# driskai/scenario_gym

Measured on NVIDIA B200. Metric: entity-steps/s, batched rollout+collision, higher is better.
Workload: dtype f64

## Files before the change

### scenario_gym_b200/csrc/sg_common.cuh

```cuda
#pragma once
#include <cuda_runtime.h>
#include <math.h>
#include <stdio.h>
#include <string.h>

#include "sg_device.cuh"
#include "sg_layout.h"

static __constant__ double c_ngon[64][2] = {
#include "sg_ngon.inc"
};

struct Grp {
  int n, s, M, G, W, H, QCAP, bar_id;
  unsigned mask;
  int64_t i, nm;
  double* corners;
  double* actbuf;
  double* rbox;
  unsigned corners_sh, rbox_sh;
  double* tcold;
  double* hcs;
  double* pedbuf;
  float4* pednb;
  uint16_t* nblist;
  double* boxp;
  double* egop;
  double* cold_d;
  int* cold_i;
  float4* aabb;
  uint32_t* queue;
  uint32_t* ego_now;
  uint32_t* ego_last;
  uint32_t* bits;
  int* acc;
  uint8_t* flags;
  int8_t* orient;
  uint16_t* sid;
  uint16_t* posof;
  int* sflag;
  float* skey;
  float4* tmpbox;
  int sorted;
  uint32_t* gstart;
  uint16_t* gsorted;
  uint16_t* glarge;
  int* gmisc;
};

SG_DEV void cp_async8(unsigned smem_addr, const void* gsrc) {
  asm volatile("cp.async.ca.shared.global [%0], [%1], 8;" ::"r"(smem_addr), "l"(gsrc) : "memory");
}
SG_DEV void cp_async_commit() { asm volatile("cp.async.commit_group;" ::: "memory"); }
SG_DEV void cp_async_wait_all() { asm volatile("cp.async.wait_group 0;" ::: "memory"); }

SG_DEV void group_sync(const Grp& g) {
  if (g.G <= 32) __syncwarp(g.mask);
  else asm volatile("bar.sync %0, %1;" ::"r"(g.bar_id), "r"(g.G) : "memory");
}

SG_DEV void setup_group(Grp& g, const SgScene& sc, const GroupLayout& L, unsigned char* smem,
                        int gl, int s, int n, int M = -1) {
  if (M < 0) M = sc.n_slots;
  unsigned char* base = smem + (size_t)gl * L.bytes;
  g.n = n; g.s = s; g.M = M; g.G = L.G; g.W = L.W; g.H = L.H; g.QCAP = L.QCAP;
  g.bar_id = 1 + gl;
  g.mask = 0xffffffffu;
  if (L.G < 32) g.mask = ((1u << L.G) - 1u) << ((threadIdx.x & 31) / L.G * L.G);
  g.nm = sc.plane_stride;
  g.i = (int64_t)n * M + s;
  g.corners = (double*)base;
  g.actbuf = (double*)(base + L.off_act);
  g.rbox = (double*)(base + L.off_rbox);
  g.corners_sh = (unsigned)__cvta_generic_to_shared(base);
  g.rbox_sh = g.corners_sh + (unsigned)L.off_rbox;
  g.tcold = (double*)(base + L.off_tcold);
  g.hcs = (double*)(base + L.off_hcs);
  g.pedbuf = (double*)(base + L.off_ped);
  g.pednb = (float4*)(base + L.off_pednb);
  g.nblist = (uint16_t*)(base + L.off_nbl);
  g.boxp = (double*)(base + L.off_box);
  g.egop = (double*)(base + L.off_ego);
  g.cold_d = (double*)(base + L.off_cold);
  g.cold_i = (int*)(base + L.off_cold + COLD_ND * sizeof(double));
  g.aabb = (float4*)(base + L.off_aabb);
  g.queue = (uint32_t*)(base + L.off_queue);
  g.ego_now = (uint32_t*)(base + L.off_hits);
  g.ego_last = g.ego_now + L.W;
  g.bits = (uint32_t*)(base + L.off_bits);
  g.acc = (int*)(base + L.off_acc);
  g.flags = (uint8_t*)(base + L.off_flags);
  g.orient = (int8_t*)(base + L.off_orient);
  g.sid = (uint16_t*)(base + L.off_sid);
  g.posof = (uint16_t*)(base + L.off_posof);
  g.sflag = (int*)(base + L.off_sflag);
  g.skey = (float*)(base + L.off_skey) + SG_SORT_WIN + 1;
  g.tmpbox = (float4*)(base + L.off_tmpbox);
  g.sorted = L.sorted;
  g.gstart = (uint32_t*)(base + L.off_gstart);
  g.gsorted = (uint16_t*)(base + L.off_gsorted);
  g.glarge = (uint16_t*)(base + L.off_glarge);
  g.gmisc = (int*)(base + L.off_gmisc);
}

SG_DEV double fast_rcp(double d) {
  double r;
  asm("rcp.approx.ftz.f64 %0, %1;" : "=d"(r) : "d"(d));
  double e = __fma_rn(-d, r, 1.0);
  r = __fma_rn(r, e, r);
  e = __fma_rn(-d, r, 1.0);
  return __fma_rn(r, e, r);
}

SG_DEV double fast_sqrt(double x) {
  double y;
  asm("rsqrt.approx.ftz.f64 %0, %1;" : "=d"(y) : "d"(x));
  const double hx = 0.5 * x;
  double e = __fma_rn(-hx * y, y, 0.5);
  y = __fma_rn(y, e, y);
  e = __fma_rn(-hx * y, y, 0.5);
  y = __fma_rn(y, e, y);
  double r = x * y;
  r = __fma_rn(__fma_rn(-r, r, x), 0.5 * y, r);
  return x > 0.0 ? r : 0.0;
}
SG_DEV double fnorm2(double a, double b) { return fast_sqrt(a * a + b * b); }

SG_DEV double div_r(double n, double d, double r) {
  const double q = n * r;
  const double rem = __fma_rn(-q, d, n);
  return __fma_rn(rem, r, q);
}

SG_DEV float4 make_aabb_box(double x, double y, double cs, double sn, double bw, double bl,
                            double bcx, double bcy, double ox, double oy) {
  const double xc = x + (bcx * cs - bcy * sn), yc = y + (bcx * sn + bcy * cs);
  const double hl = 0.5 * bl, hw = 0.5 * bw;
  const double m = 3.552713678800501e-15 *
                   (fabs(x) + fabs(y) + fabs(bl) + fabs(bw) + fabs(bcx) + fabs(bcy));
  const double ex = fabs(hl * cs) + fabs(hw * sn) + m, ey = fabs(hl * sn) + fabs(hw * cs) + m;
  float4 b;
  b.x = __double2float_rd(__dsub_rd(__dsub_rd(xc, ex), ox));
  b.y = __double2float_rd(__dsub_rd(__dsub_rd(yc, ey), oy));
  b.z = __double2float_ru(__dsub_ru(__dadd_ru(xc, ex), ox));
  b.w = __double2float_ru(__dsub_ru(__dadd_ru(yc, ey), oy));
  return b;
}

SG_DEV double min2(double a, double b) { return a < b ? a : b; }
SG_DEV double max2(double a, double b) { return a > b ? a : b; }
SG_DEV double clipd(double v, double lo, double hi) { return v < lo ? lo : (v > hi ? hi : v); }

static __constant__ double c_trig[12] = {
    -1.66666666666666324348e-01, 8.33333333332248946124e-03,  -1.98412698298579493134e-04,
    2.75573137070700676789e-06,  -2.50507602534068634195e-08, 1.58969099521155010221e-10,
    4.16666666666666019037e-02,  -1.38888888888741095749e-03, 2.48015872894767294178e-05,
    -2.75573143513906633035e-07, 2.08757232129817482790e-09,  -1.13596475577881948265e-11};
SG_DEV void sincos_kernel(double x, double& sn, double& cs) {
  const double z = x * x;
  const double* S = c_trig;
  const double* C = c_trig + 6;
  double r = __fma_rn(z, S[5], S[4]);
  r = __fma_rn(z, r, S[3]);
  r = __fma_rn(z, r, S[2]);
  r = __fma_rn(z, r, S[1]);
  r = __fma_rn(z, r, S[0]);
  sn = __fma_rn(x * z, r, x);
  double q = __fma_rn(z, C[5], C[4]);
  q = __fma_rn(z, q, C[3]);
  q = __fma_rn(z, q, C[2]);
  q = __fma_rn(z, q, C[1]);
  q = __fma_rn(z, q, C[0]);
  const double hz = 0.5 * z, w = 1.0 - hz;
  cs = w + (((1.0 - w) - hz) + z * (z * q));
}
static __device__ __noinline__ double2 sincos_lib(double x) {
  double2 r;
  sincos(x, &r.x, &r.y);
  return r;
}
static __device__ __noinline__ double tan_lib(double x) { return tan(x); }

SG_DEV double tan_small(double x) {
  double sn, cs;
  sincos_kernel(x, sn, cs);
  return div_r(sn, cs, fast_rcp(cs));
}
SG_DEV void sincos_fast(double x, double& sn, double& cs) {
  if (!(fabs(x) < 1.0e9)) { const double2 r = sincos_lib(x); sn = r.x; cs = r.y; return; }
  const double kd = rint(x * 0.63661977236758138);
  double r = __fma_rn(-kd, 1.5707963267948966, x);
  r = __fma_rn(-kd, 6.123233995736766e-17, r);
  r = __fma_rn(-kd, -1.4973849048591698e-33, r);
  double a, b;
  sincos_kernel(r, a, b);
  const int k = (int)kd;
  const double s0 = (k & 1) ? b : a, c0 = (k & 1) ? a : b;
  sn = (k & 2) ? -s0 : s0;
  cs = ((k + 1) & 2) ? -c0 : c0;
}

static __device__ __noinline__ bool in_buffer_band(double x, double y, double r, double qx, double qy) {
  const double a = atan2(-(qy - y), qx - x);
  double kk = a * (64.0 / (2.0 * M_PI));
  if (kk < 0.0) kk += 64.0;
  const int k0 = (int)kk;
#pragma unroll 1
  for (int j = -1; j <= 1; ++j) {
    const int k = (k0 + j) & 63, k1 = (k + 1) & 63;
    const double ax = x + r * c_ngon[k][0], ay = y + r * c_ngon[k][1];
    const double bx = x + r * c_ngon[k1][0], by = y + r * c_ngon[k1][1];
    if (orient_sign(ax, ay, bx, by, qx, qy) >= 0) return false;
  }
  return true;
}
SG_DEV bool in_buffer(double x, double y, double r, double qx, double qy) {
  const double dx = qx - x, dy = qy - y, d2 = dx * dx + dy * dy;
  const double rin = r * 0.99879545620517241 * (1.0 - 1e-9);
  if (d2 < rin * rin) return true;
  const double rout = r * (1.0 + 1e-9);
  if (d2 > rout * rout) return false;
  return in_buffer_band(x, y, r, qx, qy);
}

#define SG_AABB_TEST(hits, mb, ob, bit)                                                         \
  asm("{ .reg .pred p;\n\t"                                                                     \
      "setp.le.f32 p, %1, %2;\n\t"                                                              \
      "setp.le.and.f32 p, %3, %4, p;\n\t"                                                       \
      "setp.le.and.f32 p, %5, %6, p;\n\t"                                                       \
      "setp.le.and.f32 p, %7, %8, p;\n\t"                                                       \
      "@p or.b32 %0, %0, %9; }"                                                                  \
      : "+r"(hits)                                                                              \
      : "f"(mb.x), "f"(ob.z), "f"(ob.x), "f"(mb.z), "f"(mb.y), "f"(ob.w), "f"(ob.y), "f"(mb.w), \
        "r"(bit))

SG_DEV void stage_ped_state(const Grp& c, bool present, int etype, double x, double y, double vx,
                            double vy, double r, double ox, double oy) {
  c.flags[c.s] = (uint8_t)((present ? 1 : 0) | (etype << 1));
  c.pedbuf[c.s] = x; c.pedbuf[c.G + c.s] = y;
  c.pedbuf[2 * c.G + c.s] = vx; c.pedbuf[3 * c.G + c.s] = vy;
  float4 b = make_float4(INFINITY, INFINITY, -INFINITY, -INFINITY);
  if (present && etype == SG_ETYPE_PEDESTRIAN) {
    const double h = 0.5 * r * (1.0 + 1e-9);
    b.x = __double2float_rd(__dsub_rd(__dsub_rd(x, h), ox));
    b.y = __double2float_rd(__dsub_rd(__dsub_rd(y, h), oy));
    b.z = __double2float_ru(__dsub_ru(__dadd_ru(x, h), ox));
    b.w = __double2float_ru(__dsub_ru(__dadd_ru(y, h), oy));
  }
  c.pednb[c.s] = b;
}


struct GridPos {
  int ix, iy;
  bool large;
};

SG_DEV uint32_t grid_start(const uint32_t* gs, int cell) {
  const uint32_t w = gs[cell >> 1];
  return (cell & 1) ? (w >> 16) : (w & 0xffffu);
}

SG_DEV int grid_row_ranges(const uint32_t* gs, int ix, int iy, int dy, int beg[2], int end[2]) {
  const int row = ((iy + dy) & (SG_GRID_DIM - 1)) << SG_GRID_BITS;
  const int a = (ix - 1) & (SG_GRID_DIM - 1), b = (ix + 1) & (SG_GRID_DIM - 1);
  if (a < b) {
    beg[0] = (int)grid_start(gs, row | a); end[0] = (int)grid_start(gs, (row | b) + 1);
    return 1;
  }
  beg[0] = (int)grid_start(gs, row | a); end[0] = (int)grid_start(gs, row + SG_GRID_DIM);
  beg[1] = (int)grid_start(gs, row);     end[1] = (int)grid_start(gs, (row | b) + 1);
  return 2;
}

SG_DEV GridPos grid_build(const Grp& c, bool present, bool have_box, double x, double y, double ox,
                          double oy, double cs, double inv_cs) {
  uint32_t* gs = c.gstart;
  const int nwords = SG_GRID_CELLS / 2;
  for (int q = c.s; q <= nwords; q += c.G) gs[q] = 0;
  if (c.s == 0) c.gmisc[0] = 0;
  group_sync(c);
  GridPos g;
  g.ix = 0; g.iy = 0; g.large = false;
  int cell = 0;
  uint32_t rank = 0;
  if (present) {
    const double px = x - ox, py = y - oy;
    g.ix = __double2int_rd(px * inv_cs);
    g.iy = __double2int_rd(py * inv_cs);
    cell = ((g.iy & (SG_GRID_DIM - 1)) << SG_GRID_BITS) | (g.ix & (SG_GRID_DIM - 1));
    if (have_box) {
      const float4 bb = c.aabb[c.s];
      const double reach = fmax(fmax(px - (double)bb.x, (double)bb.z - px),
                                fmax(py - (double)bb.y, (double)bb.w - py));
      g.large = !(reach <= 0.5 * cs * (1.0 - 1e-6));
      if (g.large) {
        const int k = atomicAdd(&c.gmisc[0], 1);
        if (k < SG_GRID_LCAP) c.glarge[k] = (uint16_t)c.s;
      }
    }
    const uint32_t old = atomicAdd(&gs[cell >> 1], (cell & 1) ? 0x10000u : 1u);
    rank = (cell & 1) ? (old >> 16) : (old & 0xffffu);
  }
  group_sync(c);
  const int wpt = (nwords + c.G - 1) / c.G;
  const int w0 = c.s * wpt;
  uint32_t local = 0;
  for (int q = 0; q < wpt; ++q)
    if (w0 + q < nwords) { const uint32_t v = gs[w0 + q]; local += (v & 0xffffu) + (v >> 16); }
  const int lane = threadIdx.x & 31, wid = c.s >> 5;
  uint32_t incl = local;
#pragma unroll
  for (int d = 1; d < 32; d <<= 1) {
    const uint32_t o = __shfl_up_sync(0xffffffffu, incl, d);
    if (lane >= d) incl += o;
  }
  if (lane == 31) c.gmisc[8 + wid] = (int)incl;
  group_sync(c);
  uint32_t wt = lane < (c.G >> 5) ? (uint32_t)c.gmisc[8 + lane] : 0u, wi = wt;
#pragma unroll
  for (int d = 1; d < 32; d <<= 1) {
    const uint32_t o = __shfl_up_sync(0xffffffffu, wi, d);
    if (lane >= d) wi += o;
  }
  const uint32_t wbase = __shfl_sync(0xffffffffu, wi - wt, wid);
  const uint32_t total = __shfl_sync(0xffffffffu, wi, 31);
  uint32_t run = wbase + incl - local;
  for (int q = 0; q < wpt; ++q)
    if (w0 + q < nwords) {
      const uint32_t v = gs[w0 + q], lo = v & 0xffffu, hi = v >> 16;
      gs[w0 + q] = run | ((run + lo) << 16);
      run += lo + hi;
    }
  if (c.s == 0) gs[nwords] = total;
  group_sync(c);
  if (present)
    c.gsorted[grid_start(gs, cell) + rank] = (uint16_t)((uint32_t)c.s | (g.large ? SG_GRID_LARGE : 0u));
  group_sync(c);
  return g;
}

SG_DEV void broad_phase(const Grp& c, int parity);
SG_DEV void broad_phase_grid(const Grp& c, int parity, const GridPos& g) {
  const int nl = c.gmisc[0];
  if (nl > SG_GRID_LCAP) { broad_phase(c, parity); return; }
  const float4 mb = c.aabb[c.s];
  int* acc = c.acc + parity * ACC_N;
  auto test = [&](int o) {
    const float4 ob = c.aabb[o];
    if (mb.x <= ob.z && ob.x <= mb.z && mb.y <= ob.w && ob.y <= mb.w) {
      const int q = atomicAdd(&acc[ACC_QCOUNT], 1);
      if (q < c.QCAP) c.queue[q] = ((uint32_t)c.s << 16) | (uint32_t)o;
    }
  };
  if (!g.large) {
    for (int dy = -1; dy <= 1; ++dy) {
      int beg[2], end[2];
      const int nr = grid_row_ranges(c.gstart, g.ix, g.iy, dy, beg, end);
      for (int r = 0; r < nr; ++r)
        for (int idx = beg[r]; idx < end[r]; ++idx) {
          const uint32_t o = c.gsorted[idx];
          if (o > (uint32_t)c.s && o < SG_GRID_LARGE) test((int)o);
        }
    }
  }
  for (int k = 0; k < nl; ++k) {
    const int o = c.glarge[k];
    if (o == c.s || (g.large && o < c.s)) continue;
    test(o);
  }
}

struct NbForce {
  int valid;
  double a0, a1, b0, b1;
};
SG_DEV NbForce neighbour_force(const SgParams& p, const Grp& c, double px, double py, int o, double step_dt,
                               double sh, double ch, double sight_cos) {
  NbForce f;
  f.valid = 0; f.a0 = 0.0; f.a1 = 0.0; f.b0 = 0.0; f.b1 = 0.0;
  const double* bx = c.pedbuf;
  const double* by = c.pedbuf + c.G;
  const double* bvx = c.pedbuf + 2 * c.G;
  const double* bvy = c.pedbuf + 3 * c.G;
  const double ox = bx[o], oy = by[o];
  if (!in_buffer(px, py, p.ped_distance_threshold, ox, oy)) return f;
  f.valid = 1;
  const double ovx = bvx[o], ovy = bvy[o];
  const double vdx = ovx * ch + ovy * -sh, vdy = ovx * sh + ovy * ch;
  const double vn = fnorm2(vdx, vdy) + 0.0000000001, rvn = fast_rcp(vn);
  const double view0 = div_r(vdx, vn, rvn), view1 = div_r(vdy, vn, rvn);
  const double rx = px - ox, ry = py - oy, rn = fnorm2(rx, ry), rrn = fast_rcp(rn);
  const double vmag = fnorm2(ovx, ovy) + 0.0000000001, rvm = fast_rcp(vmag);
  const double uox = div_r(ovx, vmag, rvm), uoy = div_r(ovy, vmag, rvm);
  const double other_step = vmag * step_dt;
  const double r2x = rx - other_step * uox, r2y = ry - other_step * uoy;
  const double r2n = fnorm2(r2x, r2y) + 0.0000000001, rr2 = fast_rcp(r2n);
  const double b = (1.0 / 2) * fast_sqrt((rn + r2n) * (rn + r2n) - other_step * other_step);
  const double c0 = (1.0 / 4) * fast_rcp(b) * (rn + r2n);
  const double dbx = c0 * (div_r(rx, rn, rrn) + div_r(r2x, r2n, rr2)),
// ... 951 lines not shown
```

### scenario_gym_b200/csrc/sg_layout.h

```cpp
#pragma once
#include <stdint.h>
#include <cuda_runtime.h>

#define SG_THREADS 256
#define SG_NBCAP 12
#ifndef SG_SORT_MIN_M
#define SG_SORT_MIN_M 129
#endif
#ifndef SG_SWEEP_WIN
#define SG_SWEEP_WIN 4
#endif
#ifndef SG_SORT_WIN
#define SG_SORT_WIN 4
#endif
#ifndef SG_WARP_PAIRS
#define SG_WARP_PAIRS 6
#endif
#define SG_GRID_BITS 6
#define SG_GRID_DIM (1 << SG_GRID_BITS)
#define SG_GRID_CELLS (SG_GRID_DIM * SG_GRID_DIM)
#define SG_GRID_LCAP 64
#define SG_GRID_LARGE 0x8000u
#ifndef SG_VEH_THREADS
#define SG_VEH_THREADS 128
#endif
#ifndef SG_VEH_MINB
#define SG_VEH_MINB 4
#endif

struct GroupLayout {
  int G;
  int W;
  int H;
  int QCAP;
  int off_act, off_rbox, off_tcold, off_hcs, off_ped, off_pednb, off_nbl, off_box, off_ego, off_cold, off_aabb, off_queue, off_hits, off_bits,
      off_acc, off_flags, off_orient;
  int sorted;
  int off_sid, off_posof, off_sflag, off_skey, off_tmpbox;
  int grid;
  int off_gstart, off_gsorted, off_glarge, off_gmisc;
  int bytes;
};

enum { EGO_X = 0, EGO_Y, EGO_C, EGO_S, EGO_INV0, EGO_INV1, EGO_HD0, EGO_HD1, EGO_HINV0, EGO_HINV1,
       EGO_V0, EGO_V1, EGO_VNORM, EGO_VLONG, EGO_W, EGO_L, EGO_RHW, EGO_RHL, EGO_PRESENT, EGO_N = 20 };
enum { COLD_AVG = 0, COLD_AVG_T, COLD_MAX, COLD_EGOD, COLD_T0, COLD_T1, COLD_PT0, COLD_PT1, COLD_LEN,
       COLD_OX, COLD_OY, COLD_R2MINA, COLD_ND = 12 };
enum { COLD_FIRST_TICK = 0, COLD_FP0, COLD_FP1, COLD_RSS, COLD_PAIR_TICKS = 4, COLD_HAS_VEH = 6, COLD_NI = 8 };
enum { ACC_NPAIRS = 0, ACC_FIRST_PAIR, ACC_FIRST_HIT, ACC_RSS, ACC_QCOUNT, ACC_OFFROAD, ACC_N = 8 };

__host__ __device__ constexpr GroupLayout make_layout(int M, bool ped, bool rss, bool veh, bool grid = false) {
  GroupLayout L{};
  int G = 1;
  if (M <= 32) { while (G < M) G <<= 1; } else { G = (M + 31) / 32 * 32; }
  L.G = G;
  L.W = (M + 31) / 32;
  L.H = M / 2;
  L.QCAP = 4 * G;
  L.sorted = (veh && M >= SG_SORT_MIN_M && G > SG_VEH_THREADS) ? 1 : 0;
  int o = (L.sorted ? 2 : 1) * 8 * G * (int)sizeof(double);
  L.off_act = o;    o += veh ? 4 * G * (int)sizeof(double) : 0;
  L.off_rbox = o;   o += rss ? 8 * G * (int)sizeof(double) : 0;
  L.off_tcold = o;  o += veh ? 6 * G * (int)sizeof(double) : 0;
  L.off_hcs = o;    o += rss ? 2 * G * (int)sizeof(double) : 0;
  L.off_ped = o;    o += ped ? 4 * G * (int)sizeof(double) : 0;
  L.off_pednb = o;  o += ped ? (G + 32) * (int)sizeof(float4) : 0;
  L.off_nbl = o;    o += ped ? SG_NBCAP * G * (int)sizeof(uint16_t) : 0;
  o = (o + 15) / 16 * 16;
  L.off_box = o;    o += 4 * G * (int)sizeof(double);
  L.off_ego = o;    o += EGO_N * (int)sizeof(double);
  L.off_cold = o;   o += COLD_ND * (int)sizeof(double) + COLD_NI * (int)sizeof(int);
  L.off_aabb = o;   o += (M + L.H + 1) * (int)sizeof(float4);
  L.off_queue = o;  o += L.QCAP * (int)sizeof(uint32_t);
  L.off_hits = o;   o += 2 * L.W * (int)sizeof(uint32_t);
  L.off_bits = o;   o += 2 * L.W * (int)sizeof(uint32_t);
  L.off_acc = o;    o += 2 * ACC_N * (int)sizeof(int);
  L.off_flags = o;  o += G + 16;
  L.off_orient = o; o += G;
  o = (o + 15) / 16 * 16;
  L.off_sid = o;    o += L.sorted ? (M + 64) * (int)sizeof(uint16_t) : 0;
  L.off_posof = o;  o += L.sorted ? G * (int)sizeof(uint16_t) : 0;
  o = (o + 15) / 16 * 16;
  L.off_sflag = o;  o += L.sorted ? 4 * (int)sizeof(int) : 0;
  L.off_skey = o;   o += L.sorted ? (M + 2 * SG_SORT_WIN + 2) * (int)sizeof(float) : 0;
  o = (o + 15) / 16 * 16;
  L.off_tmpbox = o; o += L.sorted ? G * (int)sizeof(float4) : 0;
  L.grid = (grid && ped && G > SG_THREADS) ? 1 : 0;
  L.off_gstart = o;  o += L.grid ? (SG_GRID_CELLS / 2 + 4) * (int)sizeof(uint32_t) : 0;
  L.off_gsorted = o; o += L.grid ? G * (int)sizeof(uint16_t) : 0;
  L.off_glarge = o;  o += L.grid ? SG_GRID_LCAP * (int)sizeof(uint16_t) : 0;
  L.off_gmisc = o;   o += L.grid ? 40 * (int)sizeof(int) : 0;
  L.bytes = (o + 15) / 16 * 16;
  return L;
}
```

### scenario_gym_b200/csrc/sg_vehicle.cuh

```cuda
#pragma once
#include "sg_common.cuh"
#include "sg_internal.h"
#include "sg_pcg.cuh"

SG_DEV void cp_async4(unsigned smem_addr, const void* gsrc) {
  asm volatile("cp.async.ca.shared.global [%0], [%1], 4;" ::"r"(smem_addr), "l"(gsrc) : "memory");
}

template <bool RSS, int MC>
struct VehLayout {
  static constexpr GroupLayout value = make_layout(MC > 0 ? MC : 64, false, RSS, true, false);
};
template <bool RSS, int MAXT, int MINB, bool SORTED, bool LEAN = false, int ACT = ACT_F64, int MC = 0>
__global__ void __launch_bounds__(MAXT, MINB)
sg_vehicle_kernel(SgScene sc, SgParams p, SgState st, SgInputs in, int n_ticks, GroupLayout Lrt, SgRngDev rng) {
  extern __shared__ __align__(16) unsigned char smem[];
  const GroupLayout L = MC > 0 ? VehLayout<RSS, MC>::value : Lrt;
  const int G = L.G, M = MC > 0 ? MC : sc.n_slots, W = L.W;
  const int gpb = blockDim.x / G;
  const int gl = threadIdx.x / G;
  const int s = threadIdx.x - gl * G;
  const int n = blockIdx.x * gpb + gl;
  if (gl >= gpb || n >= sc.n_scenarios) return;
  Grp c;
  setup_group(c, sc, L, smem, gl, s, n, M);
  const bool live = s < M && sc.kind[c.i] == SG_KIND_VEHICLE;
  const int ego_slot = sc.ego_slot[n], first_slot = sc.first_slot[n];
  const bool need_coll = LEAN || (p.features & SG_FEAT_COLLISIONS) ||
                         (p.terminal & (SG_TERM_COLLISION | SG_TERM_EGO_COLLISION));
  const bool feat_rss = RSS;
  const bool matrix = !LEAN && (p.features & SG_FEAT_COLL_MATRIX) != 0;
  const bool lag = LEAN && SORTED && !(p.terminal & (SG_TERM_COLLISION | SG_TERM_EGO_COLLISION));

  double x = 0, y = 0, h = 0, vx = 0, vy = 0, dist = 0, speed = 0, cs = 1, sn = 0;
  int orient_hint = 0;
  bool present = false;
  uint8_t collided = 0, rss_state = 0, rss_last = SG_RSS_NONE;
  bool rss_evald = false;
  double* tc = c.tcold + s;
  {
    const int64_t i = c.i, nm = c.nm;
    if (live) {
      x = st.pose[i]; y = st.pose[nm + i]; h = st.pose[3 * nm + i];
      vx = st.vel[i]; vy = st.vel[nm + i];
      dist = st.dist[i]; speed = st.speed[i];
      present = st.present[i] != 0;
      collided = st.collided[i];
      sincos_fast(h, sn, cs);
      const double bw = sc.box[i], bl = sc.box[nm + i];
      c.boxp[s] = bw; c.boxp[G + s] = bl;
      c.boxp[2 * G + s] = sc.box[2 * nm + i]; c.boxp[3 * G + s] = sc.box[3 * nm + i];
      tc[4 * G] = st.vel[3 * nm + i];
      tc[5 * G] = 1.0 / bl;
      orient_hint = box_orientation_hint(bw, bl);
      if (RSS) {
        rss_state = st.rss_state[i]; rss_last = st.rss_last[i];
        tc[0] = st.safe_dist[i]; tc[G] = st.safe_dist[nm + i];
        tc[2 * G] = st.safe_ratio[i]; tc[3 * G] = st.safe_ratio[nm + i];
      }
    }
    if (s == 0) {
      double* U = c.cold_d;
      U[COLD_T0] = st.t[n]; U[COLD_PT0] = st.prev_t[n];
      U[COLD_LEN] = sc.length[n];
      const int64_t er = sc.traj_off[(int64_t)n * M + ego_slot];
      U[COLD_OX] = __ldg(sc.traj_rows + er * 7 + 1);
      U[COLD_OY] = __ldg(sc.traj_rows + er * 7 + 2);
      U[COLD_R2MINA] = 1.0 / (2 * p.rss_min_long_accel);
    }
  }
  int tick = st.tick[n];
  bool done = st.done[n] != 0;
  load_cold(st, c, n, s, W, ego_slot);
  if (RSS && s == ego_slot) publish_ego_box(c);
  if (SORTED) sorted_setup(c);
  int sort_round = 0;
  group_sync(c);

  int limit = n_ticks < 0 ? p.max_ticks : n_ticks;
  if (limit > in.n_action_ticks) limit = in.n_action_ticks;
  int parity = 0;
  const int tick0 = tick;
  double* ab = c.actbuf + s;
  const unsigned ab_sh = (unsigned)__cvta_generic_to_shared(ab);
  const double* act = in.actions + c.i;
  const float* act32 = in.actions_f32 + c.i;
  unsigned long long* rq = (unsigned long long*)c.actbuf + s;
  if (ACT == ACT_RNG) {
    if (live && limit > 0) {
#pragma unroll 1
      for (int cc = 0; cc < 2; ++cc) {
        const sg_u128 q = sg_rng_slot_state(rng, cc, c.i + (int64_t)sc.scenario_base * M);
        rq[(2 * cc) * G] = (unsigned long long)q;
        rq[(2 * cc + 1) * G] = (unsigned long long)(q >> 64);
      }
    }
  } else if (ACT == ACT_F32) {
    if (live && limit > 0 && (!done || in.step_done)) { cp_async4(ab_sh, act32); cp_async4(ab_sh + G * 8, act32 + c.nm); }
    cp_async_commit();
  } else {
    if (live && limit > 0 && (!done || in.step_done)) { cp_async8(ab_sh, act); cp_async8(ab_sh + G * 8, act + c.nm); }
    cp_async_commit();
  }

  double* const corners0 = c.corners;
  const unsigned corners_sh0 = c.corners_sh;
  for (int k = 0; k < limit && (!done || in.step_done); ++k) {
    if (LEAN && lag) {
      c.corners = corners0 + parity * 8 * G;
      c.corners_sh = corners_sh0 + (unsigned)(parity * 8 * G * 8);
    }
    const double* U = c.cold_d;
    const double t = U[COLD_T0 + parity];
    const double next_t = t + p.timestep;
    const double dt = next_t - t;
    if (ACT != ACT_RNG) cp_async_wait_all();
    if (live && present) {
      double a_in, s_in;
      if (ACT == ACT_RNG) {
        const sg_u128 A = sg_u128_make(rng.a_hi, rng.a_lo), Cc = sg_u128_make(rng.c_hi, rng.c_lo);
        unsigned long long lo = rq[0], hi = rq[G];
        a_in = rng.low[0] + rng.scale[0] * sg_pcg_double(hi, lo);
        sg_u128 q = A * sg_u128_make(hi, lo) + Cc;
        rq[0] = (unsigned long long)q; rq[G] = (unsigned long long)(q >> 64);
        lo = rq[2 * G]; hi = rq[3 * G];
        s_in = rng.low[1] + rng.scale[1] * sg_pcg_double(hi, lo);
        q = A * sg_u128_make(hi, lo) + Cc;
        rq[2 * G] = (unsigned long long)q; rq[3 * G] = (unsigned long long)(q >> 64);
      } else if (ACT == ACT_F32) {
        a_in = (double)*(const float*)(ab + parity * 2 * G);
        s_in = (double)*(const float*)(ab + parity * 2 * G + G);
      } else {
        a_in = ab[parity * 2 * G];
        s_in = ab[parity * 2 * G + G];
      }
      const double accel = clipd(a_in, -p.veh_max_accel, p.veh_max_accel);
      const double steer = clipd(s_in, -p.veh_max_steer, p.veh_max_steer);
      const double dx = speed * cs, dy = speed * sn;
      const double tn = fabs(steer) <= 0.78 ? tan_small(steer) : tan_lib(steer);
      const double dh = div_r(speed * tn, c.boxp[G + s], tc[5 * G]);
      const double nx = x + dx * dt, ny = y + dy * dt, nh = h + dh * dt;
      double ns = speed + accel * dt;
      if (!p.veh_allow_reverse) ns = ns < 0.0 ? 0.0 : ns;
      if (p.veh_max_speed == p.veh_max_speed) ns = ns > p.veh_max_speed ? p.veh_max_speed : ns;
      speed = ns;
      const double rdt = fast_rcp(dt);
      const double ex = nx - x, ey = ny - y;
      vx = div_r(ex, dt, rdt); vy = div_r(ey, dt, rdt);
      tc[4 * G] = div_r(nh - h, dt, rdt);
      dist += fnorm2(ex, ey);
      x = nx; y = ny; h = nh;
      sincos_fast(h, sn, cs);
    }
    if (ACT == ACT_F64) {
      if (live && k + 1 < limit) {
        act += 2 * c.nm;
        cp_async8(ab_sh + (parity ^ 1) * 2 * G * 8, act);
        cp_async8(ab_sh + ((parity ^ 1) * 2 * G + G) * 8, act + c.nm);
      }
      cp_async_commit();
    } else if (ACT == ACT_F32) {
      if (live && k + 1 < limit) {
        act32 += 2 * c.nm;
        cp_async4(ab_sh + (parity ^ 1) * 2 * G * 8, act32);
        cp_async4(ab_sh + ((parity ^ 1) * 2 * G + G) * 8, act32 + c.nm);
      }
      cp_async_commit();
    }
    tick += 1;
    if (!LEAN && st.trace_cap > 0 && tick < st.trace_cap && s < M) {
      const int64_t i = c.i, nm = c.nm;
      st.trace_present[(int64_t)tick * nm + i] = present;
      double* tp = st.trace_pose + (int64_t)tick * 6 * nm + i;
      tp[0] = x; tp[nm] = y; tp[2 * nm] = st.pose[2 * nm + i]; tp[3 * nm] = h;
      tp[4 * nm] = st.pose[4 * nm + i]; tp[5 * nm] = st.pose[5 * nm + i];
      if (s == 0) st.trace_t[(int64_t)tick * sc.n_scenarios + n] = next_t;
    }
    if (s < M) {
      if (need_coll || feat_rss)
        publish_box<RSS, SORTED>(c, present, x, y, cs, sn, orient_hint, U[COLD_OX], U[COLD_OY]);
      if (!LEAN && matrix) {
        uint32_t* row = st.coll_mask + ((int64_t)n * M + s) * W;
        for (int w = 0; w < W; ++w) row[w] = 0;
      }
    }
    if (RSS && feat_rss && s == ego_slot) publish_ego(c, present, x, y, cs, sn, vx, vy);
    if (s == 0) {
      c.cold_d[COLD_T0 + (parity ^ 1)] = next_t;
      c.cold_d[COLD_PT0 + (parity ^ 1)] = t;
    }
    group_sync(c);
    bool resort = false;
    if (SORTED && need_coll) {
      resort = c.sflag[3] != 0;
      if (!resort) {
        if (s < M) sorted_scatter(c);
        group_sync(c);
      }
    }
    if (LEAN && lag && k > 0)
      lagged_epilogue(p, st, c, n + sc.scenario_base, s, W, G, ego_slot, parity ^ 1, tick - 1, t);
    if (live && present) {
      if (RSS && feat_rss) {
        rss_last = SG_RSS_NONE;
        rss_evald = false;
        if (next_t != 0.0 && s != ego_slot && c.egop[EGO_PRESENT] != 0.0) {
          RssConst KR;
          KR.CLR = p.rss_min_safe_clearance; KR.RT = p.rss_response_time;
          KR.MAXA = p.rss_max_long_accel; KR.MINA = p.rss_min_long_accel;
          KR.r2mina = c.cold_d[COLD_R2MINA];
          rss_last = (uint8_t)rss_hazard<!LEAN>(KR, c, x, y, vx, vy, rss_state, tc, G);
          rss_evald = true;
          const int found = (rss_state >> 2) & 3;
          if (found) atomicOr(&c.acc[parity * ACC_N + ACC_RSS], found == 2 ? 1 : 2);
        }
      }
      if (need_coll && !SORTED) broad_phase(c, parity);
    }
    if (SORTED && need_coll && !resort && s < M) broad_phase_sorted<true>(c, parity);
    group_sync(c);
    if (SORTED && need_coll && (resort || c.sflag[3] != 0)) {
      group_sync(c);
      if (s == 0) { c.sflag[3] = 0; c.acc[parity * ACC_N + ACC_QCOUNT] = 0; }
      if (s < M) { c.aabb[s] = c.tmpbox[s]; c.sid[s] = (uint16_t)s; }
      group_sync(c);
      sort_positions(c, sort_round);
      group_sync(c);
      if (s < M) broad_phase_sorted<false>(c, parity);
      group_sync(c);
    }
    if (LEAN && lag) {
      narrow_phase_lagged(p, st, c, s, G, ego_slot, first_slot, parity, live && present);
      if (c.acc[parity * ACC_N + ACC_QCOUNT] > c.QCAP) group_sync(c);
      const double ta = c.cold_d[COLD_T0 + (parity ^ 1)], dta = ta - c.cold_d[COLD_PT0 + (parity ^ 1)];
      done = (p.terminal & SG_TERM_MAX_LENGTH) && (ta + dta > c.cold_d[COLD_LEN]);
      if (s == ego_slot && (p.features & SG_FEAT_EGO_METRICS)) {
        double* m = c.cold_d;
        const double sp = fast_sqrt(vx * vx + vy * vy);
        const double w = ta > 0.0 ? div_r(m[COLD_AVG_T], ta, fast_rcp(ta)) : m[COLD_AVG_T] / ta;
        m[COLD_AVG] += (1.0 - w) * (sp - m[COLD_AVG]);
        m[COLD_AVG_T] = ta;
        m[COLD_MAX] = fmax(sp, m[COLD_MAX]);
        m[COLD_EGOD] = dist;
      }
    } else {
      done = finish_tick<true>(p, st, c, n + sc.scenario_base, s, W, G, ego_slot, first_slot, parity, tick,
                         c.cold_d[COLD_T0 + (parity ^ 1)], c.cold_d[COLD_T0 + (parity ^ 1)] - c.cold_d[COLD_PT0 + (parity ^ 1)],
                         c.cold_d[COLD_LEN], live, live && present, collided, vx, vy, 0.0, dist);
    }
    parity ^= 1;
  }
  if (LEAN && lag && tick > tick0) {
    group_sync(c);
    lagged_epilogue(p, st, c, n + sc.scenario_base, s, W, G, ego_slot, parity ^ 1, tick, c.cold_d[COLD_T0 + parity]);
    if (live && ((c.bits[s >> 5] >> (s & 31)) & 1)) collided = 1;
  }

  if (RSS && LEAN && live && present && rss_evald) rss_ratios(c, x, y, tc, G);
  if (live) {
    const int64_t i = c.i, nm = c.nm;
    st.pose[i] = x; st.pose[nm + i] = y; st.pose[3 * nm + i] = h;
    st.vel[i] = vx; st.vel[nm + i] = vy; st.vel[3 * nm + i] = tc[4 * G];
    if (tick > tick0 && present) { st.vel[2 * nm + i] = 0.0; st.vel[4 * nm + i] = 0.0; st.vel[5 * nm + i] = 0.0; }
    st.dist[i] = dist;
    st.speed[i] = speed;
    st.collided[i] = collided;
    if (RSS) {
      st.rss_state[i] = rss_state; st.rss_last[i] = rss_last;
      st.safe_dist[i] = tc[0]; st.safe_dist[nm + i] = tc[G];
      st.safe_ratio[i] = tc[2 * G]; st.safe_ratio[nm + i] = tc[3 * G];
    }
  }
  if (s == 0) {
    st.t[n] = c.cold_d[COLD_T0 + parity]; st.prev_t[n] = c.cold_d[COLD_PT0 + parity];
    st.tick[n] = tick; st.done[n] = done;
  }
  store_cold(st, c, n, s, W, ego_slot);
}

template <bool RSS>
static cudaError_t launch_vehicle_t(int n_scen, cudaStream_t s, const SgScene& sc, const SgParams& p,
                                    const SgState& st, const SgInputs& in, const SgRngDev& rng, int act,
                                    int n_ticks, const GroupLayout& L) {
  void (*kern)(SgScene, SgParams, SgState, SgInputs, int, GroupLayout, SgRngDev);
  int threads;
  const bool lean = sgi_vehicle_lean(p, st);
  if (!lean && act != ACT_F64) return cudaErrorNotSupported;
#define SG_VEH_PICK(T, B, S)                                                                   \
  (!lean ? sg_vehicle_kernel<RSS, T, B, S, false, ACT_F64>                                     \
         : act == ACT_RNG ? sg_vehicle_kernel<RSS, T, B, S, true, ACT_RNG>                     \
         : act == ACT_F32 ? sg_vehicle_kernel<RSS, T, B, S, true, ACT_F32>                     \
                          : sg_vehicle_kernel<RSS, T, B, S, true, ACT_F64>)
#define SG_VEH_PICK_M(T, B, S, MC_)                                                            \
  (act == ACT_RNG ? sg_vehicle_kernel<RSS, T, B, S, true, ACT_RNG, MC_>                        \
                  : sg_vehicle_kernel<RSS, T, B, S, true, ACT_F64, MC_>)
  const int M = sc.n_slots;
  const bool spec = lean && (act == ACT_RNG || act == ACT_F64);
  if (L.G <= SG_VEH_THREADS) {
    kern = (spec && M == 64) ? SG_VEH_PICK_M(SG_VEH_THREADS, SG_VEH_MINB, false, 64)
         : (spec && M == 128) ? SG_VEH_PICK_M(SG_VEH_THREADS, SG_VEH_MINB, false, 128)
                              : SG_VEH_PICK(SG_VEH_THREADS, SG_VEH_MINB, false);
    threads = SG_VEH_THREADS;
  } else if (L.G <= SG_THREADS) {
    kern = (spec && M == 256 && L.sorted) ? SG_VEH_PICK_M(SG_THREADS, 2, true, 256)
         : L.sorted ? SG_VEH_PICK(SG_THREADS, 2, true) : SG_VEH_PICK(SG_THREADS, 2, false);
    threads = SG_THREADS;
  }
  else { kern = L.sorted ? SG_VEH_PICK(1024, 1, true) : SG_VEH_PICK(1024, 1, false); threads = L.G; }
#undef SG_VEH_PICK
#undef SG_VEH_PICK_M
  const int gpb = threads / L.G;
  const int blocks = (n_scen + gpb - 1) / gpb;
  const size_t smem = (size_t)gpb * L.bytes;
  if (smem > 48 * 1024) {
    cudaError_t err = cudaFuncSetAttribute(kern, cudaFuncAttributeMaxDynamicSharedMemorySize, (int)smem);
    if (err != cudaSuccess) return err;
  }
  kern<<<blocks, threads, smem, s>>>(sc, p, st, in, n_ticks, L, rng);
  return cudaGetLastError();
}
```

Before: 17.20 billion.

## Cache broad-phase candidate pairs in conservative swept windows refreshed every K ticks

```diff
diff --git a/scenario_gym_b200/csrc/sg_common.cuh b/scenario_gym_b200/csrc/sg_common.cuh
--- a/scenario_gym_b200/csrc/sg_common.cuh
+++ b/scenario_gym_b200/csrc/sg_common.cuh
@@ -41,6 +41,7 @@
   int* sflag;
   float* skey;
   float4* tmpbox;
+  float4* wbox;
   int sorted;
   uint32_t* gstart;
   uint16_t* gsorted;
@@ -96,6 +97,7 @@
   g.sflag = (int*)(base + L.off_sflag);
   g.skey = (float*)(base + L.off_skey) + SG_SORT_WIN + 1;
   g.tmpbox = (float4*)(base + L.off_tmpbox);
+  g.wbox = (float4*)(base + L.off_wbox);
   g.sorted = L.sorted;
   g.gstart = (uint32_t*)(base + L.off_gstart);
   g.gsorted = (uint16_t*)(base + L.off_gsorted);
diff --git a/scenario_gym_b200/csrc/sg_layout.h b/scenario_gym_b200/csrc/sg_layout.h
--- a/scenario_gym_b200/csrc/sg_layout.h
+++ b/scenario_gym_b200/csrc/sg_layout.h
@@ -9,6 +9,9 @@
 #endif
 #ifndef SG_SWEEP_WIN
 #define SG_SWEEP_WIN 4
+#endif
+#ifndef SG_BROAD_REFRESH
+#define SG_BROAD_REFRESH 8
 #endif
 #ifndef SG_SORT_WIN
 #define SG_SORT_WIN 4
@@ -36,7 +39,7 @@
   int off_act, off_rbox, off_tcold, off_hcs, off_ped, off_pednb, off_nbl, off_box, off_ego, off_cold, off_aabb, off_queue, off_hits, off_bits,
       off_acc, off_flags, off_orient;
   int sorted;
-  int off_sid, off_posof, off_sflag, off_skey, off_tmpbox;
+  int off_sid, off_posof, off_sflag, off_skey, off_tmpbox, off_wbox;
   int grid;
   int off_gstart, off_gsorted, off_glarge, off_gmisc;
   int bytes;
@@ -85,6 +88,7 @@
   L.off_skey = o;   o += L.sorted ? (M + 2 * SG_SORT_WIN + 2) * (int)sizeof(float) : 0;
   o = (o + 15) / 16 * 16;
   L.off_tmpbox = o; o += L.sorted ? G * (int)sizeof(float4) : 0;
+  L.off_wbox = o;   o += (veh && !L.sorted && G <= SG_VEH_THREADS && SG_BROAD_REFRESH > 1) ? (M + L.H + 1) * (int)sizeof(float4) : 0;
   L.grid = (grid && ped && G > SG_THREADS) ? 1 : 0;
   L.off_gstart = o;  o += L.grid ? (SG_GRID_CELLS / 2 + 4) * (int)sizeof(uint32_t) : 0;
   L.off_gsorted = o; o += L.grid ? G * (int)sizeof(uint16_t) : 0;
diff --git a/scenario_gym_b200/csrc/sg_vehicle.cuh b/scenario_gym_b200/csrc/sg_vehicle.cuh
--- a/scenario_gym_b200/csrc/sg_vehicle.cuh
+++ b/scenario_gym_b200/csrc/sg_vehicle.cuh
@@ -5,6 +5,77 @@
 
 SG_DEV void cp_async4(unsigned smem_addr, const void* gsrc) {
   asm volatile("cp.async.ca.shared.global [%0], [%1], 4;" ::"r"(smem_addr), "l"(gsrc) : "memory");
+}
+
+static_assert(SG_BROAD_REFRESH >= 1 && SG_BROAD_REFRESH <= 256, "SG_BROAD_REFRESH: 1 .. 256 ticks");
+template <int K>
+SG_DEV void publish_window(const Grp& c, const SgParams& p, bool present, double x, double y, double speed,
+                           double t, double ox, double oy) {
+  float4 wb = make_float4(INFINITY, INFINITY, -INFINITY, -INFINITY);
+  if (present) {
+    const double hl = 0.5 * fabs(c.boxp[c.G + c.s]), hw = 0.5 * fabs(c.boxp[c.s]);
+    const double R = fnorm2(fabs(c.boxp[2 * c.G + c.s]) + hl, fabs(c.boxp[3 * c.G + c.s]) + hw);
+    const double ts = fabs(p.timestep);
+    const double dt = ts + 0x1p-50 * (fabs(t) + (K + 1) * ts);
+    const double v = fmax(fabs(speed), -p.veh_max_speed);
+    const double D = (K - 1) * v * dt + (0.5 * (K - 1) * (K - 2)) * fabs(p.veh_max_accel) * dt * dt;
+    const double e = D + R;
+    const double E = e + 0x1p-40 * (fabs(x) + fabs(y) + 4.0 * e);
+    if (E + fabs(x) + fabs(y) + fabs(speed) < INFINITY) {
+      wb.x = __double2float_rd(__dsub_rd(__dsub_rd(x, E), ox));
+      wb.y = __double2float_rd(__dsub_rd(__dsub_rd(y, E), oy));
+      wb.z = __double2float_ru(__dsub_ru(__dadd_ru(x, E), ox));
+      wb.w = __double2float_ru(__dsub_ru(__dadd_ru(y, E), oy));
+    } else {
+      wb = make_float4(-INFINITY, -INFINITY, INFINITY, INFINITY);
+    }
+  }
+  c.wbox[c.s] = wb;
+  if (c.s < c.H + 1) c.wbox[c.M + c.s] = wb;
+}
+
+template <int NW>
+SG_DEV void broad_phase_cached(const Grp& c, int parity, uint32_t (&cand)[NW], bool rebuild) {
+  const float4 mb = c.aabb[c.s];
+  int* acc = c.acc + parity * ACC_N;
+#pragma unroll
+  for (int w = 0; w < NW; ++w) {
+    const int d0 = 32 * w;
+    if (rebuild) {
+      const float4 mw = c.wbox[c.s];
+      const float4* nw = c.wbox + c.s + 1 + d0;
+      const int dn = min(32, c.H - d0);
+      uint32_t m = 0;
+      if (dn == 32) {
+#pragma unroll
+        for (int dd = 0; dd < 32; ++dd) {
+          const float4 ob = nw[dd];
+          SG_AABB_TEST(m, mw, ob, 1u << dd);
+        }
+      } else {
+        for (int dd = 0; dd < dn; ++dd) {
+          const float4 ob = nw[dd];
+          SG_AABB_TEST(m, mw, ob, 1u << dd);
+        }
+      }
+      cand[w] = m;
+    }
+    uint32_t todo = cand[w];
+    while (todo) {
+      const int dd = __ffs(todo) - 1;
+      todo &= todo - 1;
+      const int d = d0 + dd + 1;
+      const float4 ob = c.aabb[c.s + d];
+      uint32_t hit = 0;
+      SG_AABB_TEST(hit, mb, ob, 1u);
+      if (!hit) continue;
+      int j = c.s + d;
+      if (j >= c.M) j -= c.M;
+      if (2 * d == c.M && c.s > j) continue;
+      const int q = atomicAdd(&acc[ACC_QCOUNT], 1);
+      if (q < c.QCAP) c.queue[q] = ((uint32_t)c.s << 16) | (uint32_t)j;
+    }
+  }
 }
 
 template <bool RSS, int MC>
@@ -31,6 +102,9 @@
   const bool feat_rss = RSS;
   const bool matrix = !LEAN && (p.features & SG_FEAT_COLL_MATRIX) != 0;
   const bool lag = LEAN && SORTED && !(p.terminal & (SG_TERM_COLLISION | SG_TERM_EGO_COLLISION));
+  constexpr bool CACHE = LEAN && !SORTED && MAXT <= SG_VEH_THREADS && SG_BROAD_REFRESH > 1;
+  constexpr int NCW = MC > 0 ? (MC / 2 + 31) / 32 : 2;
+  uint32_t cand[NCW] = {};
 
   double x = 0, y = 0, h = 0, vx = 0, vy = 0, dist = 0, speed = 0, cs = 1, sn = 0;
   int orient_hint = 0;
@@ -179,6 +253,8 @@
     if (s < M) {
       if (need_coll || feat_rss)
         publish_box<RSS, SORTED>(c, present, x, y, cs, sn, orient_hint, U[COLD_OX], U[COLD_OY]);
+      if (CACHE && k % SG_BROAD_REFRESH == 0)
+        publish_window<SG_BROAD_REFRESH>(c, p, present, x, y, speed, next_t, U[COLD_OX], U[COLD_OY]);
       if (!LEAN && matrix) {
         uint32_t* row = st.coll_mask + ((int64_t)n * M + s) * W;
         for (int w = 0; w < W; ++w) row[w] = 0;
@@ -215,7 +291,8 @@
           if (found) atomicOr(&c.acc[parity * ACC_N + ACC_RSS], found == 2 ? 1 : 2);
         }
       }
-      if (need_coll && !SORTED) broad_phase(c, parity);
+      if (CACHE) broad_phase_cached(c, parity, cand, k % SG_BROAD_REFRESH == 0);
+      else if (need_coll && !SORTED) broad_phase(c, parity);
     }
     if (SORTED && need_coll && !resort && s < M) broad_phase_sorted<true>(c, parity);
     group_sync(c);
```

Result: faster. 17.47 billion, median of 6 (+1.6%).
